# VisualComputingInstitute/RovinaSemanticSegmentation

Hardware: AMD Instinct MI355X
Metric: Mpix/s RF+5-iter DenseCRF @640x480 RGB-D (higher is better)
Workload: dtype f32; 1 GPU; BASELINE configs[2]: batch of 64 synthetic 640x480 RGB-D key frames per GPU (10 % invalid-depth holes: yes; 2 input sets in rotation), 4-tree forest (2^14 leaves/tree, D=366, C=9), RF + 5-iter DenseCRF (d=6, Potts w=10), marginals + labels written to HBM; label_gather=none

## Files before the change

rovinasemanticsegmentation_amd/csrc/kernels_lattice.hip:

```cpp
#include <string.h>

#include <type_traits>

#include <rocprim/rocprim.hpp>

#include "device_math.h"
#include "rvseg_crf.h"

namespace rvseg {

constexpr int ST_EMPTY = -1, ST_LOCKED = -2, ST_FILLED = 0;

struct Key8 {
    union {
        short k[8];
        unsigned w[4];
        unsigned long long q[2];
    };
};

__device__ __forceinline__ unsigned hash_key(const Key8& key) {
    unsigned h = 0x9E3779B9u;
#pragma unroll
    for (int i = 0; i < 4; i++) {
        h ^= key.w[i];
        h *= 0x85EBCA6Bu;
        h ^= h >> 15;
    }
    return h;
}

__device__ __forceinline__ bool key_equal_at(const unsigned long long* tkeys, unsigned slot, const Key8& key) {
    const unsigned long long* mine = key.q;
    const unsigned long long a = __hip_atomic_load(tkeys + 2 * (size_t)slot, __ATOMIC_RELAXED, __HIP_MEMORY_SCOPE_AGENT);
    const unsigned long long b = __hip_atomic_load(tkeys + 2 * (size_t)slot + 1, __ATOMIC_RELAXED, __HIP_MEMORY_SCOPE_AGENT);
    return a == mine[0] && b == mine[1];
}

__device__ __forceinline__ unsigned hash_insert(int* state, unsigned long long* tkeys, unsigned base, unsigned mask,
                                                int* counters, const Key8& key) {
    unsigned hl = hash_key(key) & mask;
    for (unsigned probes = 0; probes <= mask; ) {
        const unsigned h = base + hl;
        int st = __hip_atomic_load(state + h, __ATOMIC_RELAXED, __HIP_MEMORY_SCOPE_AGENT);
        if (st == ST_EMPTY) {
            int expected = ST_EMPTY;
            if (__hip_atomic_compare_exchange_strong(state + h, &expected, ST_LOCKED, __ATOMIC_RELAXED, __ATOMIC_RELAXED,
                                                     __HIP_MEMORY_SCOPE_AGENT)) {
                const unsigned long long* mine = key.q;
                __hip_atomic_store(tkeys + 2 * (size_t)h, mine[0], __ATOMIC_RELAXED, __HIP_MEMORY_SCOPE_AGENT);
                __hip_atomic_store(tkeys + 2 * (size_t)h + 1, mine[1], __ATOMIC_RELAXED, __HIP_MEMORY_SCOPE_AGENT);
                __hip_atomic_store(state + h, ST_FILLED, __ATOMIC_RELEASE, __HIP_MEMORY_SCOPE_AGENT);
                return h;
            }
            continue;
        }
        if (st == ST_LOCKED) continue;
        if (key_equal_at(tkeys, h, key)) return h;
        hl = (hl + 1) & mask;
        probes++;
    }
    counters[1] = 1;
    return base;
}

__device__ __forceinline__ int hash_lookup(const int* state, const unsigned long long* tkeys, unsigned base, unsigned mask,
                                           const Key8& key) {
    unsigned hl = hash_key(key) & mask;
    const unsigned long long* mine = key.q;
    for (unsigned probes = 0; probes <= mask; probes++) {
        const unsigned h = base + hl;
        if (state[h] == ST_EMPTY) return -1;
        if (tkeys[2 * (size_t)h] == mine[0] && tkeys[2 * (size_t)h + 1] == mine[1]) return (int)h;
        hl = (hl + 1) & mask;
    }
    return -1;
}

constexpr int LP_SET = 512;
constexpr int LP_MAX_PROBE = 24;
constexpr int LP_CHUNKS = 8;

template <int D, bool NARROW = false>
__global__ void __launch_bounds__(256)
lattice_points_kernel(LatticeDev L, FeatureSource fs, int n_chunks) {
    __shared__ int ltag[LP_SET];
    __shared__ unsigned long long lkey[LP_SET][2];
    __shared__ unsigned lslot[LP_SET];
    __shared__ unsigned short lnew[LP_SET];
    __shared__ unsigned n_new;
    for (int t = threadIdx.x; t < LP_SET; t += 256) ltag[t] = ST_EMPTY;
    if (threadIdx.x == 0) n_new = 0;
    __syncthreads();
    const int lane = threadIdx.x & 63;
    unsigned resolved = 0;
    const long long per_frame = L.Npad;

  for (int chunk = 0; chunk < n_chunks; chunk++) {
    const long long gid0 = ((long long)blockIdx.x * n_chunks + chunk) * 256 + threadIdx.x;
    const bool active = gid0 < per_frame * L.n_frames;
    const long long gid = active ? gid0 : 0;
    const int frame = (int)(gid / per_frame);
    const int i = (int)(gid - (long long)frame * per_frame);
    const bool real = active && i < L.N;
    const long long gp = (long long)frame * L.N + i;

    float f[D];
    if (!real) {
#pragma unroll
        for (int k = 0; k < D; k++) f[k] = 0.0f;
    } else if (fs.mode == 0) {
#pragma unroll
        for (int k = 0; k < D; k++) f[k] = fs.feat[gp * D + k];
    } else {
        const float4 c = fs.cloud[gp];
        float x = c.x, y = c.y, z = c.z;
        if (!(finite_f(x) && finite_f(y) && finite_f(z))) x = y = z = 0.0f;
        const uint8_t* px = fs.rgb + gp * 3;
        const float v[6] = {x * fs.xyz_kernel, y * fs.xyz_kernel, z * fs.xyz_kernel,
                            ((float)px[0] / 255.0f) * fs.rgb_kernel, ((float)px[1] / 255.0f) * fs.rgb_kernel,
                            ((float)px[2] / 255.0f) * fs.rgb_kernel};
#pragma unroll
        for (int k = 0; k < D; k++) f[k] = v[k < 6 ? k : 0];
    }

    const float invdplus1 = 1.0f / (D + 1), dplus1 = (float)(D + 1);
    float el[D + 1], rem0[D + 1], rank[D + 1];
    float sm = 0.0f;
#pragma unroll
    for (int j = D; j > 0; j--) {
        const float cf = f[j - 1] * L.scale[j - 1];
        el[j] = sm - (float)j * cf;
        sm += cf;
    }
    el[0] = sm;
    float sum = 0.0f;
#pragma unroll
    for (int k = 0; k <= D; k++) {
        float v = invdplus1 * el[k];
        v = rintf(v);
        rem0[k] = v * dplus1;
        sum += v;
    }
#pragma unroll
    for (int k = 0; k <= D; k++) rank[k] = 0.0f;
#pragma unroll
    for (int a = 0; a < D; a++) {
        const float di = el[a] - rem0[a];
#pragma unroll
        for (int b = a + 1; b <= D; b++) {
            const float dj = el[b] - rem0[b];
            const float c = di < dj ? 1.0f : 0.0f;
            rank[a] += c;
            rank[b] += 1.0f - c;
        }
    }
#pragma unroll
    for (int k = 0; k <= D; k++) {
        rank[k] += sum;
        const float add = rank[k] < 0.0f ? dplus1 : 0.0f;
        const float sub = rank[k] >= dplus1 ? dplus1 : 0.0f;
        rank[k] += add - sub;
        rem0[k] += add - sub;
    }
    float bary[D + 2];
#pragma unroll
    for (int k = 0; k < D + 2; k++) bary[k] = 0.0f;
#pragma unroll
    for (int k = 0; k <= D; k++) {
        const float v = (el[k] - rem0[k]) * invdplus1;
        const int p = D - (int)rank[k];
#pragma unroll
        for (int q = 0; q <= D; q++) {
            if (q == p) { bary[q] += v; bary[q + 1] -= v; }
        }
    }
    bary[0] += 1.0f + bary[D + 1];
    int lidx[D + 1];
#pragma unroll
    for (int r = 0; r <= D; r++) {
        Key8 key;
#pragma unroll
        for (int k = 0; k < 8; k++) key.k[k] = 0;
#pragma unroll
        for (int k = 0; k < D; k++) {
            const int rk = (int)rank[k];
            const int canon = rk <= D - r ? r : r - (D + 1);
            key.k[k] = (short)(rem0[k] + (float)canon);
        }
        key.k[7] = (short)frame;
        int leader_of = lane;
        {
            bool pending = active;
            for (;;) {
                const unsigned long long todo = __ballot(pending);
                if (!todo) break;
                const int ld = __ffsll((long long)todo) - 1;
                const unsigned a0 = __builtin_amdgcn_readlane(key.w[0], ld), a1 = __builtin_amdgcn_readlane(key.w[1], ld);
                const unsigned a2 = __builtin_amdgcn_readlane(key.w[2], ld), a3 = __builtin_amdgcn_readlane(key.w[3], ld);
                const bool same = pending && key.w[0] == a0 && key.w[1] == a1 && key.w[2] == a2 && key.w[3] == a3;
                if (same) leader_of = ld;
                pending = pending && !same;
            }
        }
        int found = 0;
        if (active && leader_of == lane) {
            unsigned h = (hash_key(key) >> 7) & (LP_SET - 1);
            found = -1;
            for (int probes = 0; probes < LP_MAX_PROBE; ) {
                const int t = __hip_atomic_load(&ltag[h], __ATOMIC_RELAXED, __HIP_MEMORY_SCOPE_WORKGROUP);
                if (t == ST_EMPTY) {
                    int expected = ST_EMPTY;
                    if (__hip_atomic_compare_exchange_strong(&ltag[h], &expected, ST_LOCKED, __ATOMIC_RELAXED, __ATOMIC_RELAXED,
                                                             __HIP_MEMORY_SCOPE_WORKGROUP)) {
                        __hip_atomic_store(&lkey[h][0], key.q[0], __ATOMIC_RELAXED, __HIP_MEMORY_SCOPE_WORKGROUP);
                        __hip_atomic_store(&lkey[h][1], key.q[1], __ATOMIC_RELAXED, __HIP_MEMORY_SCOPE_WORKGROUP);
                        __hip_atomic_store(&ltag[h], ST_FILLED, __ATOMIC_RELEASE, __HIP_MEMORY_SCOPE_WORKGROUP);
                        lnew[atomicAdd(&n_new, 1u)] = (unsigned short)h;
                        found = (int)h;
                        break;
                    }
                    continue;
                }
                if (t == ST_LOCKED) continue;
                const unsigned long long a = __hip_atomic_load(&lkey[h][0], __ATOMIC_RELAXED, __HIP_MEMORY_SCOPE_WORKGROUP);
                const unsigned long long b = __hip_atomic_load(&lkey[h][1], __ATOMIC_RELAXED, __HIP_MEMORY_SCOPE_WORKGROUP);
                if (a == key.q[0] && b == key.q[1]) { found = (int)h; break; }
                h = (h + 1) & (LP_SET - 1);
                probes++;
            }
            if (found < 0)
                found = -1 - (int)hash_insert(L.state, L.tkeys, (unsigned)frame << L.cap_f_log2, L.cap_f_mask, L.counters, key);
        }
        lidx[r] = __shfl(found, leader_of, 64);
    }
    __syncthreads();
    const unsigned created = n_new;
    for (unsigned t = resolved + threadIdx.x; t < created; t += 256) {
        const unsigned h = lnew[t];
        Key8 key;
        key.q[0] = lkey[h][0];
        key.q[1] = lkey[h][1];
        const unsigned fr = (unsigned)(unsigned short)key.k[7];
        lslot[h] = hash_insert(L.state, L.tkeys, fr << L.cap_f_log2, L.cap_f_mask, L.counters, key);
    }
    resolved = created;
    __syncthreads();
    if (real) {
        int so[D + 1];
#pragma unroll
        for (int r = 0; r <= D; r++) {
            const int li = lidx[r];
            so[r] = li >= 0 ? (int)lslot[li] : -1 - li;
            if (NARROW) so[r] &= (int)L.cap_f_mask;
        }
        if constexpr (NARROW) store_ids16(L.offsets, (size_t)gp, so);
        else store_row<D + 1>(L.offsets + gp * (D + 1), so);
        store_row<D + 1>(L.bary + gp * (D + 1), bary);
    }
  }
}

template <class F>
static void with_dimension(int d, F&& f) {
    switch (d) {
        case 1: f(std::integral_constant<int, 1>()); break;
        case 2: f(std::integral_constant<int, 2>()); break;
        case 3: f(std::integral_constant<int, 3>()); break;
        case 4: f(std::integral_constant<int, 4>()); break;
        case 5: f(std::integral_constant<int, 5>()); break;
        case 6: f(std::integral_constant<int, 6>()); break;
        case 7: f(std::integral_constant<int, 7>()); break;
        default: break;
    }
}

void launch_lattice_points(const LatticeDev& L, const FeatureSource& fs, hipStream_t s) {
    const long long total = (long long)L.Npad * L.n_frames;
    int n_chunks = LP_CHUNKS;
    while (n_chunks > 1 && (total + 255) / 256 / n_chunks < 1024) n_chunks >>= 1;
    const long long per_block = 256ll * n_chunks;
    const dim3 grid((unsigned)((total + per_block - 1) / per_block)), block(256);
    with_dimension(L.d, [&](auto dim) {
        constexpr int D = decltype(dim)::value;
        if constexpr (D == 6) {
            if (L.ids16) { lattice_points_kernel<6, true><<<grid, block, 0, s>>>(L, fs, n_chunks); return; }
        }
        lattice_points_kernel<D><<<grid, block, 0, s>>>(L, fs, n_chunks);
    });
    RV_LAUNCHED("lattice_points_kernel");
}

struct SlotFilled {
    __device__ __forceinline__ int operator()(int st) const { return st == ST_FILLED ? 1 : 0; }
};

__global__ void __launch_bounds__(256)
lattice_compact_kernel(LatticeDev L) {
    const unsigned slot = blockIdx.x * blockDim.x + threadIdx.x;
    if (slot >= L.cap_total) return;
    const bool filled = L.state[slot] == ST_FILLED;
    const int id = L.slot_to_id[slot];
    if (filled && (unsigned)id < (unsigned)L.m_bound) {
        L.vkeys[2 * (size_t)id] = L.tkeys[2 * (size_t)slot];
        L.vkeys[2 * (size_t)id + 1] = L.tkeys[2 * (size_t)slot + 1];
    }
    const unsigned cap_f = L.cap_f_mask + 1;
    if ((slot & L.cap_f_mask) == 0) L.fstart[slot >> L.cap_f_log2] = id;
    if (slot == L.cap_total - 1) {
        const int M = id + (filled ? 1 : 0);
        L.counters[0] = M;
        L.fstart[L.n_frames] = M;
        if (M > L.m_bound) L.counters[1] = 1;
    }
    if ((slot & L.cap_f_mask) == L.cap_f_mask) {
        const int first = L.slot_to_id[slot - L.cap_f_mask];
        const int Mf = id + (filled ? 1 : 0) - first;
        if ((unsigned)Mf > cap_f / 2) L.counters[1] = 1;
    }
}

__global__ void __launch_bounds__(256)
lattice_remap_kernel(LatticeDev L, unsigned* __restrict__ sort_keys, unsigned* __restrict__ sort_vals, long long n_entries) {
    const long long e = (long long)blockIdx.x * blockDim.x + threadIdx.x;
    if (e >= n_entries) return;
    int id = L.slot_to_id[L.offsets[e]];
    id = id < L.m_bound ? id : L.m_bound - 1;
    L.offsets[e] = id;
    sort_keys[e] = (unsigned)id;
    sort_vals[e] = (unsigned)e;
}

__global__ void __launch_bounds__(256)
lattice_neighbours_kernel(LatticeDev L) {
    const long long gid = (long long)blockIdx.x * blockDim.x + threadIdx.x;
    const int M = L.counters[0] < L.m_bound ? L.counters[0] : L.m_bound;
    const int d = L.d;
    if (gid >= (long long)M * (d + 1)) return;
    const int j = (int)(gid / M);
    const int id = (int)(gid - (long long)j * M);
    Key8 key;
    const unsigned long long* src = L.vkeys + 2 * (size_t)id;
    key.q[0] = src[0];
    key.q[1] = src[1];
    Key8 n1 = key, n2 = key;
    for (int k = 0; k < d; k++) { n1.k[k] = (short)(key.k[k] - 1); n2.k[k] = (short)(key.k[k] + 1); }
    if (j < d) { n1.k[j] = (short)(key.k[j] + d); n2.k[j] = (short)(key.k[j] - d); }
    const unsigned fbase = (unsigned)(unsigned short)key.k[7] << L.cap_f_log2;
    const int s1 = hash_lookup(L.state, L.tkeys, fbase, L.cap_f_mask, n1);
    const int s2 = hash_lookup(L.state, L.tkeys, fbase, L.cap_f_mask, n2);
    L.nb1[(size_t)j * L.m_bound + id] = s1 < 0 ? -1 : L.slot_to_id[s1];
    L.nb2[(size_t)j * L.m_bound + id] = s2 < 0 ? -1 : L.slot_to_id[s2];
}

__global__ void __launch_bounds__(256)
lattice_csr_kernel(LatticeDev L, const unsigned* __restrict__ keys_sorted, const unsigned* __restrict__ vals_sorted,
                   long long n_entries) {
    const long long k = (long long)blockIdx.x * blockDim.x + threadIdx.x;
    if (k >= n_entries) return;
    const unsigned e = vals_sorted[k];
    const unsigned key = keys_sorted[k];
    L.csr_pw[k] = make_uint2(e / (unsigned)(L.d + 1), __float_as_uint(L.bary[e]));
    if (k == 0 || keys_sorted[k - 1] != key) L.vstart[key] = (unsigned)k;
    if (k == n_entries - 1 || keys_sorted[k + 1] != key) L.vend[key] = (unsigned)(k + 1);
}

void launch_vertex_order(const LatticeDev& L, SortBuffers& sb, hipStream_t s);

constexpr int CS_PIX_MIN = 256;
constexpr int CS_MCAP = 4096;

struct CsLaunch {
    int mcap, wbpf;
    dim3 grid, block;
    size_t lds;
};
static CsLaunch cs_launch(const LatticeDev& L) {
    CsLaunch c;
    c.mcap = (int)((L.cap_f_mask + 1) / 2);
    c.wbpf = (L.N + L.cs_pix - 1) / L.cs_pix;
    c.grid = dim3((unsigned)(((long long)c.wbpf * L.n_frames + 3) / 4));
    c.block = dim3(256);
    c.lds = (size_t)4 * c.mcap * sizeof(unsigned);
    return c;
}

__device__ __forceinline__ int2 cs_frame_vertices(const LatticeDev& L, int frame, int mcap) {
    const int2 fr = lattice_frame_range(L, frame, L.m_bound);
    return make_int2(fr.x, fr.y - fr.x < mcap ? fr.y - fr.x : mcap);
}

struct CsWaveBlock {
    bool outside;
    int lane, frame, wb;
    int f0, Mf;
    long long p0, p1;
    long long ebeg, eend;
    unsigned* my;
    size_t row;
};
__device__ __forceinline__ CsWaveBlock cs_wave_block(const LatticeDev& L, int wbpf, int mcap) {
    extern __shared__ unsigned cs_cnt[];
    CsWaveBlock B{};
    const int wave = threadIdx.x >> 6;
    const long long gwb = (long long)blockIdx.x * 4 + wave;
    B.lane = threadIdx.x & 63;
    B.frame = (int)(gwb / wbpf);
    B.outside = B.frame >= L.n_frames;
    if (B.outside) return B;
    B.wb = (int)(gwb - (long long)B.frame * wbpf);
    const int2 fv = cs_frame_vertices(L, B.frame, mcap);
    B.f0 = fv.x;
    B.Mf = fv.y;
    B.p0 = (long long)B.wb * L.cs_pix;
    B.p1 = B.p0 + L.cs_pix < L.N ? B.p0 + L.cs_pix : L.N;
    B.ebeg = ((long long)B.frame * L.N + B.p0) * (L.d + 1);
    B.eend = ((long long)B.frame * L.N + B.p1) * (L.d + 1);
    B.my = cs_cnt + (size_t)wave * mcap;
    B.row = (size_t)wbpf * B.f0 + (size_t)B.wb * B.Mf;
    return B;
}

__device__ __forceinline__ void load_unit(const int* p, int (&v)[4]) { load_row<4>(p, v); }
__device__ __forceinline__ void store_unit(int* p, const int (&v)[4]) { store_row<4>(p, v); }
__device__ __forceinline__ void load_unit(const u16_ids* p, int (&v)[8]) {
    const u16x8_ids t = *reinterpret_cast<const u16x8_ids*>(p);
#pragma unroll
    for (int k = 0; k < 8; k++) v[k] = t[k];
}
__device__ __forceinline__ void store_unit(u16_ids* p, const int (&v)[8]) {
    u16x8_ids t;
#pragma unroll
    for (int k = 0; k < 8; k++) t[k] = (unsigned short)v[k];
    *reinterpret_cast<u16x8_ids*>(p) = t;
}

template <bool NARROW>
__global__ void __launch_bounds__(256)
csr_count_kernel(LatticeDev L, unsigned* __restrict__ bh, int wbpf, int mcap) {
    constexpr int W = NARROW ? 8 : 4;
    typedef typename std::conditional<NARROW, u16_ids, int>::type id_t;
    const CsWaveBlock B = cs_wave_block(L, wbpf, mcap);
    if (B.outside) return;
    const int lane = B.lane, f0 = B.f0, Mf = B.Mf;
    const long long ebeg = B.ebeg, eend = B.eend;
    unsigned* my = B.my;
    for (int lv = lane; lv < Mf; lv += 64) my[lv] = 0u;
    __builtin_amdgcn_fence(__ATOMIC_SEQ_CST, "wavefront");
    const long long ubeg = NARROW ? ebeg & ~7ll : ebeg;
    id_t* ids = reinterpret_cast<id_t*>(L.offsets);
    const int* s2i = L.slot_to_id + (NARROW ? (size_t)B.frame << L.cap_f_log2 : (size_t)0);
    auto mine = [&](long long e) { return (!NARROW || e >= ebeg) && e < eend; };
    auto whole = [&](long long e) { return (!NARROW || e >= ebeg) && e + W <= eend; };
    auto fetch = [&](long long e, int (&sl)[W]) {
        if (whole(e)) {
            load_unit(ids + e, sl);
        } else {
#pragma unroll
            for (int k = 0; k < W; k++) sl[k] = mine(e + k) ? (int)ids[e + k] : 0;
        }
    };
    int sl_n[W];
    fetch(ubeg + W * lane < eend ? ubeg + W * lane : ubeg, sl_n);
    for (long long base = ubeg; base < eend; base += 64 * W) {
        const long long e = base + W * lane;
        int sl[W], id[W], lv[W];
#pragma unroll
        for (int k = 0; k < W; k++) sl[k] = sl_n[k];
        const bool any = e < eend;
        if (any) {
#pragma unroll
            for (int k = 0; k < W; k++) id[k] = s2i[sl[k]];
        }
        const long long en = e + 64 * W;
        fetch(en < eend ? en : ubeg, sl_n);
        if (!any) continue;
#pragma unroll
        for (int k = 0; k < W; k++) {
            id[k] = id[k] < L.m_bound ? id[k] : L.m_bound - 1;
            lv[k] = id[k] - f0;
            lv[k] = lv[k] < Mf ? lv[k] : Mf - 1;
            lv[k] = lv[k] < 0 ? 0 : lv[k];
        }
        const int (&out)[W] = NARROW ? lv : id;
        if (whole(e)) {
            store_unit(ids + e, out);
        } else {
#pragma unroll
            for (int k = 0; k < W; k++) if (mine(e + k)) ids[e + k] = (id_t)out[k];
        }
#pragma unroll
        for (int k = 0; k < W; k++) {
            if (mine(e + k) && Mf > 0) atomicAdd(&my[lv[k]], 1u);
        }
    }
    __builtin_amdgcn_fence(__ATOMIC_SEQ_CST, "wavefront");
    unsigned* row = bh + B.row;
    for (int lv = lane; lv < Mf; lv += 64) row[lv] = my[lv];
}

template <int DP1, bool NARROW = false>
__global__ void __launch_bounds__(256)
csr_scatter_kernel(LatticeDev L, const unsigned* __restrict__ bh, int wbpf, int mcap) {
    const CsWaveBlock B = cs_wave_block(L, wbpf, mcap);
    if (B.outside) return;
    const int lane = B.lane, frame = B.frame, f0 = B.f0, Mf = B.Mf;
    const unsigned n_entries_total = (unsigned)((long long)L.n_frames * L.N * DP1);
    unsigned* my = B.my;
    const unsigned* row = bh + B.row;
    for (int lv = lane; lv < Mf; lv += 64) my[lv] = row[lv];
    if (Mf == 0 && lane == 0) my[0] = 0xFFFFFFFFu;
    __builtin_amdgcn_fence(__ATOMIC_SEQ_CST, "wavefront");
    const int p0 = (int)B.p0, p1 = (int)B.p1;
    const unsigned long long lt = lane == 0 ? 0ull : (~0ull >> (64 - lane));
    for (int pc = p0; pc < p1; pc += 64) {
        const int p = pc + lane;
        const bool valid = p < p1;
        const size_t gp = (size_t)frame * L.N + (valid ? p : p1 - 1);
        int lv[DP1];
        float w[DP1];
        if constexpr (NARROW) {
            unsigned raw[4];
            load_ids16(L.offsets, gp, raw);
            unpack_ids16(raw, gp, lv);
        } else {
            load_row<DP1>(L.offsets + gp * DP1, lv);
        }
        load_row<DP1>(L.bary + gp * DP1, w);
#pragma unroll
        for (int j = 0; j < DP1; j++) {
            if (!NARROW) lv[j] -= f0;
            lv[j] = lv[j] < Mf ? lv[j] : Mf - 1;
            lv[j] = lv[j] < 0 ? 0 : lv[j];
        }
        unsigned pend = valid ? (1u << DP1) - 1u : 0u;
#pragma unroll
        for (int j = 0; j < DP1; j++) {
            for (;;) {
                const unsigned long long todo = __ballot((pend >> j) & 1u);
                if (!todo) break;
                const int leader = __ffsll((long long)todo) - 1;
                const int k = __builtin_amdgcn_readlane(lv[j], leader);
                unsigned long long all = 0ull;
                float wsel = 0.0f;
                bool hit = false;
#pragma unroll
                for (int jj = j; jj < DP1; jj++) {
                    const bool same = ((pend >> jj) & 1u) && lv[jj] == k;
                    all |= __ballot(same);
                    if (same) { wsel = w[jj]; hit = true; pend &= ~(1u << jj); }
                }
                const unsigned b = my[k];
                if (hit) {
                    const unsigned pos = b + (unsigned)__popcll(all & lt);
                    if (pos < n_entries_total) L.csr_pw[pos] = make_uint2((unsigned)gp, __float_as_uint(wsel));
                }
                if (lane == leader) my[k] = b + (unsigned)__popcll(all);
            }
        }
        __builtin_amdgcn_fence(__ATOMIC_SEQ_CST, "wavefront");
    }
}

__global__ void __launch_bounds__(256)
csr_scatter_entries_kernel(LatticeDev L, const unsigned* __restrict__ bh, int wbpf, int mcap) {
    const CsWaveBlock B = cs_wave_block(L, wbpf, mcap);
    if (B.outside) return;
    const int lane = B.lane, f0 = B.f0, Mf = B.Mf, dp1 = L.d + 1;
    const long long ebeg = B.ebeg, eend = B.eend;
    const unsigned n_entries_total = (unsigned)((long long)L.n_frames * L.N * dp1);
    unsigned* my = B.my;
    const unsigned* row = bh + B.row;
    for (int lv = lane; lv < Mf; lv += 64) my[lv] = row[lv];
    if (Mf == 0 && lane == 0) my[0] = 0xFFFFFFFFu;
    __builtin_amdgcn_fence(__ATOMIC_SEQ_CST, "wavefront");
    const unsigned long long lt = lane == 0 ? 0ull : (~0ull >> (64 - lane));
    auto fetch = [&](long long e, int& id, float& wgt) {
        id = 0; wgt = 0.f;
        if (e < eend) { id = L.offsets[e]; wgt = L.bary[e]; }
    };
    int id_n; float w_n;
    fetch(ebeg + lane, id_n, w_n);
    for (long long base = ebeg; base < eend; base += 64) {
        const long long e = base + lane;
        const bool valid = e < eend;
        const int id = id_n;
        const float wgt = w_n;
        fetch(e + 64, id_n, w_n);
        int lv = valid ? id - f0 : -1;
        if (lv >= Mf) lv = Mf - 1;
        if (valid && lv < 0) lv = 0;
        bool pending = valid;
        for (;;) {
            const unsigned long long todo = __ballot(pending);
            if (!todo) break;
            const int leader = __ffsll((long long)todo) - 1;
            const int k = __shfl(lv, leader, 64);
            const bool same = pending && lv == k;
            const unsigned long long m = __ballot(same);
            const unsigned b = my[k];
            if (same) {
                const unsigned pos = b + (unsigned)__popcll(m & lt);
                if (pos < n_entries_total) L.csr_pw[pos] = make_uint2((unsigned)(e / dp1), __float_as_uint(wgt));
            }
            if (lane == leader) my[k] = b + (unsigned)__popcll(m);
            pending = pending && !same;
        }
        __builtin_amdgcn_fence(__ATOMIC_SEQ_CST, "wavefront");
    }
}

constexpr int CS_SEGS = 16;
__device__ __forceinline__ size_t csr_aux_offset(const LatticeDev& L, int wbpf) { return (size_t)wbpf * ((size_t)L.m_bound + 64); }

__global__ void __launch_bounds__(1024)
csr_total_kernel(LatticeDev L, unsigned* __restrict__ bh, int wbpf, int mcap, int n_groups) {
    __shared__ unsigned sseg[CS_SEGS][64];
    const int frame = blockIdx.x / n_groups, grp = blockIdx.x - frame * n_groups;
    const int2 fv = cs_frame_vertices(L, frame, mcap);
    const int f0 = fv.x, Mf = fv.y;
    const int lv0 = grp * 64;
    if (lv0 >= Mf) return;
    const int lvl = threadIdx.x & 63, seg = threadIdx.x >> 6;
    const int sw = (wbpf + CS_SEGS - 1) / CS_SEGS;
    const int w0 = seg * sw, w1 = (w0 + sw < wbpf) ? w0 + sw : wbpf;
    const unsigned* fb = bh + (size_t)wbpf * f0;
    unsigned* vtot = bh + csr_aux_offset(L, wbpf);
    unsigned* segsum = vtot + L.m_bound;
    const int lv = lv0 + lvl;
    const bool ok = lv < Mf;
    unsigned sum = 0;
    if (ok) for (int w = w0; w < w1; w++) sum += fb[(size_t)w * Mf + lv];
    sseg[seg][lvl] = sum;
    if (ok) segsum[(size_t)(f0 + lv) * CS_SEGS + seg] = sum;
    __syncthreads();
    if (seg == 0 && ok) {
        unsigned total = 0;
#pragma unroll
        for (int q = 0; q < CS_SEGS; q++) total += sseg[q][lvl];
        vtot[f0 + lv] = total;
    }
}

__global__ void __launch_bounds__(1024)
csr_scan_kernel(LatticeDev L, unsigned* __restrict__ bh, int wbpf, int mcap, int n_groups) {
    __shared__ unsigned red[16];
    __shared__ unsigned vbase[64];
    const int frame = blockIdx.x / n_groups, grp = blockIdx.x - frame * n_groups;
    const int2 fv = cs_frame_vertices(L, frame, mcap);
    const int f0 = fv.x, Mf = fv.y;
    const int lv0 = grp * 64;
    if (lv0 >= Mf) return;
    const int lvl = threadIdx.x & 63, seg = threadIdx.x >> 6;
    const int sw = (wbpf + CS_SEGS - 1) / CS_SEGS;
    const int w0 = seg * sw, w1 = (w0 + sw < wbpf) ? w0 + sw : wbpf;
    unsigned* fb = bh + (size_t)wbpf * f0;
    const unsigned* vtot = bh + csr_aux_offset(L, wbpf);
    const unsigned* segsum = vtot + L.m_bound;
    const unsigned frame_base = (unsigned)((long long)frame * L.N * (L.d + 1));
    unsigned part = 0;
    for (int v = threadIdx.x; v < lv0; v += 1024) part += vtot[f0 + v];
    for (int off = 32; off > 0; off >>= 1) part += __shfl_xor(part, off, 64);
    if (lvl == 0) red[seg] = part;
    __syncthreads();
    unsigned carry = 0;
#pragma unroll
    for (int q = 0; q < 16; q++) carry += red[q];
    const int lv = lv0 + lvl;
    const bool ok = lv < Mf;
    if (seg == 0) {
        const unsigned total = ok ? vtot[f0 + lv] : 0u;
        unsigned incl = total;
        for (int off = 1; off < 64; off <<= 1) {
            const unsigned t = __shfl_up(incl, off, 64);
            if (lvl >= off) incl += t;
        }
        vbase[lvl] = carry + incl - total;
        if (ok) {
            L.vstart[f0 + lv] = frame_base + carry + incl - total;
            L.vend[f0 + lv] = frame_base + carry + incl;
        }
    }
    __syncthreads();
    if (ok) {
        unsigned run = frame_base + vbase[lvl];
        for (int q = 0; q < seg; q++) run += segsum[(size_t)(f0 + lv) * CS_SEGS + q];
        for (int w = w0; w < w1; w++) {
            const unsigned t = fb[(size_t)w * Mf + lv];
            fb[(size_t)w * Mf + lv] = run;
            run += t;
        }
    }
}

bool csr_fast_path(const LatticeDev& L) { return ((L.cap_f_mask + 1) / 2) <= (unsigned)CS_MCAP; }
size_t csr_fast_bytes(const LatticeDev& L) {
    const size_t wbpf = (size_t)cs_launch(L).wbpf;
    return (wbpf * ((size_t)L.m_bound + 64) + (size_t)L.m_bound * (1 + CS_SEGS)) * sizeof(unsigned);
}

void launch_csr_scatter(const LatticeDev& L, SortBuffers& sb, hipStream_t s) {
    if (!(csr_fast_path(L) && sb.block_hist)) return;
    const CsLaunch c = cs_launch(L);
    with_dimension(L.d, [&](auto dim) {
        constexpr int DP1 = decltype(dim)::value + 1;
        if constexpr (DP1 == 7) {
            if (L.ids16) { csr_scatter_kernel<7, true><<<c.grid, c.block, c.lds, s>>>(L, sb.block_hist, c.wbpf, c.mcap); return; }
        }
        if constexpr (DP1 == 3 || DP1 == 6 || DP1 == 7)
            csr_scatter_kernel<DP1><<<c.grid, c.block, c.lds, s>>>(L, sb.block_hist, c.wbpf, c.mcap);
        else
            csr_scatter_entries_kernel<<<c.grid, c.block, c.lds, s>>>(L, sb.block_hist, c.wbpf, c.mcap);
    });
    RV_LAUNCHED("csr_scatter_kernel");
}

void launch_lattice_finish(const LatticeDev& L, SortBuffers& sb, long long n_entries, hipStream_t s, bool defer_scatter) {
    const unsigned cap = L.cap_total;
    {
        size_t temp = sb.scan_temp_bytes;
        auto in = rocprim::make_transform_iterator(L.state, SlotFilled());
        (void)rocprim::exclusive_scan(sb.scan_temp, temp, in, L.slot_to_id, 0, (size_t)cap, rocprim::plus<int>(), s);
    }
    lattice_compact_kernel<<<dim3((cap + 255) / 256), dim3(256), 0, s>>>(L);
    const long long nb_threads = (long long)L.m_bound * (L.d + 1);
    lattice_neighbours_kernel<<<dim3((unsigned)((nb_threads + 255) / 256)), dim3(256), 0, s>>>(L);
    RV_LAUNCHED("lattice_compact_kernel / lattice_neighbours_kernel");
    if (csr_fast_path(L) && sb.block_hist) {
        const CsLaunch c = cs_launch(L);
        if (L.ids16) csr_count_kernel<true><<<c.grid, c.block, c.lds, s>>>(L, sb.block_hist, c.wbpf, c.mcap);
        else csr_count_kernel<false><<<c.grid, c.block, c.lds, s>>>(L, sb.block_hist, c.wbpf, c.mcap);
        const int n_groups = (c.mcap + 63) / 64;
        csr_total_kernel<<<dim3((unsigned)(L.n_frames * n_groups)), dim3(1024), 0, s>>>(L, sb.block_hist, c.wbpf, c.mcap, n_groups);
        csr_scan_kernel<<<dim3((unsigned)(L.n_frames * n_groups)), dim3(1024), 0, s>>>(L, sb.block_hist, c.wbpf, c.mcap, n_groups);
        RV_LAUNCHED("csr_count_kernel / csr_total_kernel / csr_scan_kernel");
        if (!defer_scatter) launch_csr_scatter(L, sb, s);
    } else {
        lattice_remap_kernel<<<dim3((unsigned)((n_entries + 255) / 256)), dim3(256), 0, s>>>(L, sb.keys_in, sb.vals_in, n_entries);
        size_t temp = sb.temp_bytes;
        (void)rocprim::radix_sort_pairs(sb.temp, temp, sb.keys_in, sb.keys_out, sb.vals_in, sb.vals_out, (size_t)n_entries, 0,
                                        (unsigned)sb.key_bits, s);
        lattice_csr_kernel<<<dim3((unsigned)((n_entries + 255) / 256)), dim3(256), 0, s>>>(L, sb.keys_out, sb.vals_out, n_entries);
        RV_LAUNCHED("lattice_remap_kernel / radix sort / lattice_csr_kernel");
    }
    launch_vertex_order(L, sb, s);
}

__global__ void __launch_bounds__(256)
vertex_len_kernel(LatticeDev L, unsigned* __restrict__ key, unsigned* __restrict__ ids, int len_shift) {
    const int v = blockIdx.x * blockDim.x + threadIdx.x;
    if (v >= L.m_bound) return;
    const int M = L.counters[0] < L.m_bound ? L.counters[0] : L.m_bound;
    unsigned k = 0xFFFFFFFFu;
    if (v < M) {
        atomicMax(&L.counters[3], (int)(L.vend[v] - L.vstart[v]));
        const unsigned len = (L.vend[v] - L.vstart[v]) >> len_shift;
        const unsigned frame = (unsigned)(unsigned short)(L.vkeys[2 * (size_t)v + 1] >> 48);
        k = ((frame < 1023u ? frame : 1022u) << 22) | (0x3FFFFFu - (len < 0x3FFFFFu ? len : 0x3FFFFFu));
    }
    key[v] = k;
    ids[v] = (unsigned)v;
}

void launch_vertex_order(const LatticeDev& L, SortBuffers& sb, hipStream_t s) {
    int len_shift = 0;
    while (((long long)L.N >> len_shift) >= (1 << 22)) len_shift++;
    vertex_len_kernel<<<dim3((unsigned)((L.m_bound + 255) / 256)), dim3(256), 0, s>>>(L, sb.keys_in, sb.vals_in, len_shift);
    size_t temp = sb.temp_bytes;
    (void)rocprim::radix_sort_pairs(sb.temp, temp, sb.keys_in, sb.keys_out, sb.vals_in, L.vorder, (size_t)L.m_bound, 0, 32, s);
    RV_LAUNCHED("vertex_len_kernel / radix sort");
}

size_t scan_temp_bytes(unsigned cap) {
    size_t temp = 0;
    int* nul = nullptr;
    auto in = rocprim::make_transform_iterator(nul, SlotFilled());
    (void)rocprim::exclusive_scan(nullptr, temp, in, nul, 0, (size_t)cap, rocprim::plus<int>(), (hipStream_t)0);
    return temp;
}

size_t sort_temp_bytes(long long n_entries, int key_bits) {
    size_t temp = 0;
    unsigned* nul = nullptr;
    (void)rocprim::radix_sort_pairs(nullptr, temp, nul, nul, nul, nul, (size_t)n_entries, 0, (unsigned)key_bits, (hipStream_t)0);
    return temp;
}

__global__ void __launch_bounds__(256)
csr_norm_kernel(const uint2* __restrict__ csr_pw, const float* __restrict__ norm, float* __restrict__ csr_nrm, long long n_entries,
                const int* __restrict__ counters) {
    if (counters[1]) return;
    const long long k = (long long)blockIdx.x * blockDim.x + threadIdx.x;
    if (k < n_entries) csr_nrm[k] = norm[csr_pw[k].x];
}

void launch_csr_norm(const LatticeDev& L, long long n_entries, hipStream_t s) {
    csr_norm_kernel<<<dim3((unsigned)((n_entries + 255) / 256)), dim3(256), 0, s>>>(L.csr_pw, L.norm, L.csr_nrm, n_entries, L.counters);
    RV_LAUNCHED("csr_norm_kernel");
}
int csr_pix_min() { return CS_PIX_MIN; }

}
```

Baseline: 1808 Mpix/s.

## Prefetch next chunk and defer CSR scatter writes out of ballot loop

Software-pipelines the CSR scatter kernel so the next 64-point chunk's offsets and barycentric weights are loaded while the current chunk is processed. The ballot dedup loop now only records per-vertex ranks and group totals. The shared-counter reads, global CSR stores and counter updates happen afterwards in one unrolled pass. This aims to hide load latency and take LDS reads and scattered global stores off the serial leader loop, at the cost of more registers, an extra prefetch past the end, and rank/total packed into 8-bit fields.

```diff
diff --git a/rovinasemanticsegmentation_amd/csrc/kernels_lattice.hip b/rovinasemanticsegmentation_amd/csrc/kernels_lattice.hip
--- a/rovinasemanticsegmentation_amd/csrc/kernels_lattice.hip
+++ b/rovinasemanticsegmentation_amd/csrc/kernels_lattice.hip
@@ -502,6 +502,7 @@
 template <int DP1, bool NARROW = false>
 __global__ void __launch_bounds__(256)
 csr_scatter_kernel(LatticeDev L, const unsigned* __restrict__ bh, int wbpf, int mcap) {
+    constexpr int RW = NARROW ? 4 : DP1;
     const CsWaveBlock B = cs_wave_block(L, wbpf, mcap);
     if (B.outside) return;
     const int lane = B.lane, frame = B.frame, f0 = B.f0, Mf = B.Mf;
@@ -513,26 +514,43 @@
     __builtin_amdgcn_fence(__ATOMIC_SEQ_CST, "wavefront");
     const int p0 = (int)B.p0, p1 = (int)B.p1;
     const unsigned long long lt = lane == 0 ? 0ull : (~0ull >> (64 - lane));
+    auto point = [&](int pc) {
+        const int p = pc + lane;
+        return (unsigned)frame * (unsigned)L.N + (unsigned)(p < p1 ? p : p1 - 1);
+    };
+    auto fetch = [&](size_t gp, unsigned (&raw)[RW], float (&w)[DP1]) {
+        if constexpr (NARROW) load_ids16(L.offsets, gp, raw);
+        else load_row<DP1>(reinterpret_cast<const unsigned*>(L.offsets) + gp * DP1, raw);
+        load_row<DP1>(L.bary + gp * DP1, w);
+    };
+    unsigned raw_n[RW];
+    float w_n[DP1];
+    unsigned gp_n = point(p0);
+    fetch(gp_n, raw_n, w_n);
     for (int pc = p0; pc < p1; pc += 64) {
-        const int p = pc + lane;
-        const bool valid = p < p1;
-        const size_t gp = (size_t)frame * L.N + (valid ? p : p1 - 1);
+        const bool valid = pc + lane < p1;
+        const unsigned gp = gp_n;
         int lv[DP1];
         float w[DP1];
         if constexpr (NARROW) {
-            unsigned raw[4];
-            load_ids16(L.offsets, gp, raw);
-            unpack_ids16(raw, gp, lv);
+            unpack_ids16(raw_n, gp, lv);
         } else {
-            load_row<DP1>(L.offsets + gp * DP1, lv);
-        }
-        load_row<DP1>(L.bary + gp * DP1, w);
+#pragma unroll
+            for (int j = 0; j < DP1; j++) lv[j] = (int)raw_n[j];
+        }
+#pragma unroll
+        for (int j = 0; j < DP1; j++) w[j] = w_n[j];
+        gp_n = point(pc + 64);
+        fetch(gp_n, raw_n, w_n);
 #pragma unroll
         for (int j = 0; j < DP1; j++) {
             if (!NARROW) lv[j] -= f0;
             lv[j] = lv[j] < Mf ? lv[j] : Mf - 1;
             lv[j] = lv[j] < 0 ? 0 : lv[j];
         }
+        unsigned rt[DP1];
+#pragma unroll
+        for (int j = 0; j < DP1; j++) rt[j] = 0u;
         unsigned pend = valid ? (1u << DP1) - 1u : 0u;
 #pragma unroll
         for (int j = 0; j < DP1; j++) {
@@ -542,21 +560,36 @@
                 const int leader = __ffsll((long long)todo) - 1;
                 const int k = __builtin_amdgcn_readlane(lv[j], leader);
                 unsigned long long all = 0ull;
-                float wsel = 0.0f;
-                bool hit = false;
+                unsigned hit = 0u;
 #pragma unroll
                 for (int jj = j; jj < DP1; jj++) {
                     const bool same = ((pend >> jj) & 1u) && lv[jj] == k;
                     all |= __ballot(same);
-                    if (same) { wsel = w[jj]; hit = true; pend &= ~(1u << jj); }
+                    if (same) hit |= 1u << jj;
                 }
-                const unsigned b = my[k];
-                if (hit) {
-                    const unsigned pos = b + (unsigned)__popcll(all & lt);
-                    if (pos < n_entries_total) L.csr_pw[pos] = make_uint2((unsigned)gp, __float_as_uint(wsel));
+                const unsigned r = (unsigned)__popcll(all & lt);
+#pragma unroll
+                for (int jj = j; jj < DP1; jj++) {
+                    if ((hit >> jj) & 1u) rt[jj] = r;
                 }
-                if (lane == leader) my[k] = b + (unsigned)__popcll(all);
+                pend &= ~hit;
+                if (lane == leader) rt[j] |= (unsigned)__popcll(all) << 8;
             }
+        }
+        unsigned base[DP1];
+#pragma unroll
+        for (int j = 0; j < DP1; j++) base[j] = my[lv[j]];
+        if (valid) {
+#pragma unroll
+            for (int j = 0; j < DP1; j++) {
+                const unsigned pos = base[j] + (rt[j] & 0xFFu);
+                if (pos < n_entries_total) L.csr_pw[pos] = make_uint2(gp, __float_as_uint(w[j]));
+            }
+        }
+#pragma unroll
+        for (int j = 0; j < DP1; j++) {
+            const unsigned total = rt[j] >> 8;
+            if (total) my[lv[j]] = base[j] + total;
         }
         __builtin_amdgcn_fence(__ATOMIC_SEQ_CST, "wavefront");
     }
```

New measurement: 1829 Mpix/s (median of 6 runs). 1.2% higher.
